# AnnSeidel/genometools

Measured on AMD Instinct MI355X. Metric: Gbp/s ESA build (suf+lcp+bwt), 3 Gbp DNA, 1/2/4/8 MI355X; bit-exact vs CPU, higher is better.
Workload: dtype u64; 1 GPU; human-like DNA (2% N, 24 seqs, repeats) n=3000000000 seed=43 -suf -lcp -bwt (BASELINE.json configs[2]); parallelism=1 device, pair_suffixes=341032298, tied_suffixes=390540711, refine_rounds=9, maxbranchdepth=8256

## Files before the change

genometools_amd/_lib.py:

```python
import ctypes
import os
import subprocess

HERE = os.path.dirname(os.path.abspath(__file__))
ROOT = os.path.dirname(HERE)
LIB_PATH = os.path.join(HERE, "libgtamd_esa.so")
SOURCES = [os.path.join(HERE, "csrc", f) for f in
           ("esa_prims.hip", "esa_engine.hip", "esa_synth.hip", "esa_encode.hip",
            "esa_pck.hip", "esa_comm.hip")]
HEADERS = [os.path.join(HERE, "csrc", f) for f in ("esa_common.h", "esa_prims.h", "esa_devutil.h", "esa_msd.h",
                                                     "esa_pck_replay.h")] + \
          [os.path.join(ROOT, "include", h) for h in ("gtamd_esa.h", "gtamd_encode.h", "gtamd_pck.h")]
HIPCC = os.environ.get("HIPCC", "/opt/rocm/bin/hipcc")


def needs_build():
    if not os.path.exists(LIB_PATH):
        return True
    t = os.path.getmtime(LIB_PATH)
    return any(os.path.getmtime(p) > t for p in SOURCES + HEADERS)


def build_library(force=False, verbose=False):
    if not force and not needs_build():
        return LIB_PATH
    cmd = [HIPCC, "--offload-arch=gfx950", "-O3", "-std=c++17", "-fPIC",
           "-shared", "-Wall", "-Wno-unused-function", "-o", LIB_PATH] + SOURCES
    if verbose:
        print(" ".join(cmd))
    subprocess.run(cmd, check=True)
    return LIB_PATH


class EsaStats(ctypes.Structure):
    _fields_ = [("totallength", ctypes.c_uint64),
                ("numberofallsortedsuffixes", ctypes.c_uint64),
                ("longest", ctypes.c_uint64),
                ("largelcpvalues", ctypes.c_uint64),
                ("maxbranchdepth", ctypes.c_uint64),
                ("lcptabsum", ctypes.c_uint64),
                ("prefixlength", ctypes.c_uint32),
                ("refine_rounds", ctypes.c_uint32),
                ("tied_suffixes", ctypes.c_uint64),
                ("pair_suffixes", ctypes.c_uint64),
                ("device_bytes", ctypes.c_uint64),
                ("msd_big_entries", ctypes.c_uint64),
                ("msd_crowded_entries", ctypes.c_uint64),
                ("rank_entries_built", ctypes.c_uint64)]


class EsaTiming(ctypes.Structure):
    _fields_ = [("total_ms", ctypes.c_float),
                ("keygen_ms", ctypes.c_float),
                ("sort_ms", ctypes.c_float),
                ("finalize_ms", ctypes.c_float),
                ("refine_ms", ctypes.c_float),
                ("tie_fix_ms", ctypes.c_float),
                ("scatter_ms", ctypes.c_float),
                ("scatter_launches", ctypes.c_uint32),
                ("scatter_items", ctypes.c_uint64),
                ("comm_ms", ctypes.c_float),
                ("comm_calls", ctypes.c_uint32),
                ("comm_bytes", ctypes.c_uint64),
                ("alloc_ms", ctypes.c_float),
                ("dominant_kernel", ctypes.c_uint32),
                ("scatter_read_items", ctypes.c_uint64),
                ("scatter_written_items", ctypes.c_uint64)]


class EncodeSummary(ctypes.Structure):
    _fields_ = [(name, ctypes.c_uint64) for name in
                ("totallength", "numofsequences", "specialcharacters",
                 "realspecialranges")] + \
               [("specialrangestab", ctypes.c_uint64 * 3)] + \
               [(name, ctypes.c_uint64) for name in
                ("lengthofspecialprefix", "lengthofspecialsuffix", "wildcards",
                 "realwildcardranges")] + \
               [("wildcardrangestab", ctypes.c_uint64 * 3)] + \
               [(name, ctypes.c_uint64) for name in
                ("lengthofwildcardprefix", "lengthofwildcardsuffix",
                 "lengthoflongestnonspecial", "minseqlen", "maxseqlen",
                 "equallength")] + \
               [("characterdistribution", ctypes.c_uint64 * 32),
                ("originaldistribution", ctypes.c_uint64 * 256)]


class PckParams(ctypes.Structure):
    _fields_ = [("block_size", ctypes.c_uint32), ("bucket_blocks", ctypes.c_uint32),
                ("locate_interval", ctypes.c_uint32), ("feature_toggles", ctypes.c_int32),
                ("with_statistics", ctypes.c_int32)]


class PckInfo(ctypes.Structure):
# ... 115 lines not shown
```

genometools_amd/csrc/esa_engine.hip:

```cpp
#include <stdarg.h>
#include <stdlib.h>
#include <chrono>
#include <functional>
#include <type_traits>
#include <vector>
#include "../../include/gtamd_esa.h"
#include "esa_prims.h"
#include "esa_devutil.h"

static thread_local char g_err[1024] = "";
void gtamd_set_error(const char *fmt, ...) {
  va_list ap;
  va_start(ap, fmt);
  vsnprintf(g_err, sizeof g_err, fmt, ap);
  va_end(ap);
}
extern "C" const char *gtamd_esa_last_error(void) { return g_err; }

extern "C" int gtamd_device_count(void) {
  GTAMD_ABI_BEGIN
  int n = 0;
  if (hipGetDeviceCount(&n) != hipSuccess) return 0;
  return n;
  GTAMD_ABI_END(0)
// ... 2901 lines not shown
  if (m == 0) return 0;
  const u64 nb = div_up(m, 256);
  k_dest_place<F><<<(u32) nb, 256, 0, c->st>>>(f, m, c->numparts, nb, dest, boff);
  HIP_TRY(hipGetLastError());
  return 0;
}
static u64 dest_words(u32 R, u64 m) { return (u64) R * div_up(m ? m : 1, 256) + 16; }

template <int BITS>
static int build_bcktab(gtamd_esa_ctx *c, const u64 *skey, const u32 *spos, u64 NL, u32 k,
                        hipStream_t st) {
  u64 codes = 1, special = 1, dist = 0, pw = 1;
  for (u32 j = 0; j < k; j++) {
    if (codes > (1ull << 31) / c->sigma) {
      gtamd_set_error("bucket table for prefixlength %u over %u letters is too "
                      "large", k, c->sigma);
      return -1;
    }
    codes *= c->sigma;
  }
  for (u32 j = 0; j + 1 < k; j++) special *= c->sigma;
  for (u32 j = 1; j + 1 < k; j++) { pw *= c->sigma; dist += pw; }
  const u64 total = codes + 1 + special + dist;
  free_dev(c->bck);
  c->bck = nullptr;
  HIP_TRY(hipMalloc(&c->bck, total * 4));
  HIP_TRY(hipMemsetAsync(c->bck, 0, total * 4, st));
  if (NL > 0) {
    k_bck_count<BITS><<<(u32) div_up(NL, 256), 256, 0, st>>>(
        skey, NL, k, c->sigma, c->bck, c->bck + codes + 1,
        c->bck + codes + 1 + special, c->text, spos);
    HIP_TRY(hipGetLastError());
  }
  u32 *ws = c->rws.as<u32>();
  u32 *own = nullptr;
  if (scan_workspace_words(codes + 1) * 4 > c->rws.bytes) {
    HIP_TRY(hipMalloc(&own, scan_workspace_words(codes + 1) * 4));
    ws = own;
  }
  const int rc = scan_u32(SCAN_SUM, c->bck, c->bck, codes + 1, false, ws, st);
  if (own != nullptr) { (void) hipStreamSynchronize(st); free_dev(own); }
  TRY(rc);
  c->bck_codes = codes; c->bck_special = special; c->bck_dist = dist;
  return 0;
}

static u64 rws_words_for(u64 cap) {
  return radix_workspace_words(cap) + 10 * (div_up(cap, 64) + 64) +
         scan_workspace_words(div_up(cap, 64)) + 64;
}
static int ensure_workspace(gtamd_esa_ctx *c, u64 cap, u32 want, bool dist) {
  const u64 pad = cap + 8;
  TRY(ensure_buf(c, c->k0, pad * 8, "sort keys"));
  TRY(ensure_buf(c, c->k1, pad * 8, "sort keys"));
  TRY(ensure_buf(c, c->v0, pad * 4, "sort values"));
  TRY(ensure_buf(c, c->v1, pad * 4, "sort values"));
  TRY(ensure_buf(c, c->rws, rws_words_for(cap) * 4, "the radix workspace"));
  TRY(ensure_buf(c, c->tiebits, (div_up(cap, 64) + 2) * 8, "the tie bitmap"));
  if (want & GTAMD_WANT_SUF) TRY(ensure_buf(c, c->suf, pad * 8, "the suffix table"));
  if (want & GTAMD_WANT_LCP) TRY(ensure_buf(c, c->lcp, pad, "the lcp table"));
  if (want & GTAMD_WANT_BWT) TRY(ensure_buf(c, c->bwt, pad, "the bwt table"));
  if (dist) TRY(ensure_buf(c, c->isa_tmp, pad * 8, "the exchange scratch"));
  return 0;
}

static int msd_cbits_max(u64 N) {
  const int c = bits_for(N > 1 ? N - 1 : 1) - 24;
  return c < 0 ? 0 : (c > 8 ? 8 : c);
}
static int msd_choose_cbits(u64 N, int cmax, const float *penalty) {
  int best = cmax;
  float best_cost = 0.0f;
  for (int k = 1; k >= 0; k--) {
    const int c = cmax - 2 + k;
    if (c < 6) continue;
    const float gain = k == 1 ? 0.17f : 0.57f;
    const float cost = (penalty[k] - penalty[2]) / (float) N - gain;
    if (cost < best_cost) { best = c; best_cost = cost; }
  }
  return best;
}
struct MsdWs {
  u32 *hist, *scanws, *tcnt, *tfirst, *dtcnt, *dtfirst, *startA, *startB, *F, *scan2, *counters,
      *biglist, *giantlist, *crowdlist;
  MsTile *desc;
  MdTile *dtiles;
  u64 *firstkey, *lastkey;
  u32 rows, tilesB_ub, tilesC_ub, tilesD_ub;
  u64 nf;
};
static u64 msd_carve(u64 N, int cb, u8 *base, MsdWs *w) {
  const u32 ntA = (u32) div_up(N, MS_TILE);
  w->tilesB_ub = ntA + 256;
  w->tilesC_ub = ntA + MSD_PARENTS;
  w->tilesD_ub = (u32) (2 * div_up(N, MS_TILE)) + MSD_PARENTS + 8;
  w->rows = w->tilesC_ub + 2;
  w->nf = (u64) MSD_PARENTS << cb;
  Bump b;
  b.base = base;
  b.off = 0;
  w->hist = b.take<u32>((u64) w->rows * 256);
  w->scanws = b.take<u32>(radix_rows_workspace_words(w->rows));
  w->desc = b.take<MsTile>(w->tilesC_ub);
  w->tcnt = b.take<u32>(MSD_PARENTS + 8);
  w->tfirst = b.take<u32>(MSD_PARENTS + 8);
  w->dtcnt = b.take<u32>(MSD_PARENTS + 8);
  w->dtfirst = b.take<u32>(MSD_PARENTS + 8);
  w->startA = b.take<u32>(256 + 8);
  w->startB = b.take<u32>(MSD_PARENTS + 8);
  w->F = b.take<u32>(w->nf + 8);
  w->scan2 = b.take<u32>(scan_workspace_words(w->nf + 1) + 64);
  w->counters = b.take<u32>(16);
  w->dtiles = b.take<MdTile>(w->tilesD_ub);
  w->firstkey = b.take<u64>(w->tilesD_ub);
  w->lastkey = b.take<u64>(w->tilesD_ub);
  w->biglist = b.take<u32>(w->tilesD_ub);
  w->crowdlist = b.take<u32>(w->tilesD_ub);
  w->giantlist = b.take<u32>((u64) (N / MS_TILE) + 8);
  return b.off + 256;
}

static int msd_level_prepare(gtamd_esa_ctx *c, const MsdWs &w, const u32 *pstart, u32 np, int cb,
                             u32 tiles_ub, const u32 *kin, u32 *cstart) {
  hipStream_t st = c->st;
  k_msd_tilecount<<<(np + 1 + 255) / 256, 256, 0, st>>>(pstart, 0, np, (u32) MS_TILE, w.tcnt);
  HIP_TRY(hipGetLastError());
  TRY(scan_u32(SCAN_SUM, w.tcnt, w.tfirst, (u64) np + 1, false, w.scan2, st));
  k_msd_tiledesc<<<(tiles_ub + 255) / 256, 256, 0, st>>>(pstart, w.tfirst, np, tiles_ub, w.desc);
  HIP_TRY(hipGetLastError());
  k_msd_hist_lvl<<<tiles_ub + 1, MS_THREADS, 0, st>>>(kin, w.desc, tiles_ub, 32 - cb, w.hist);
  HIP_TRY(hipGetLastError());
  TRY(radix_scan_tile_rows(w.hist, tiles_ub + 1, w.scanws, st));
  const u64 nchild = (u64) np << cb;
  k_msd_tot<<<(u32) div_up(nchild + 1, 256), 256, 0, st>>>(w.hist, w.tfirst, np, cb, cstart);
  HIP_TRY(hipGetLastError());
  TRY(scan_u32(SCAN_SUM, cstart, cstart, nchild + 1, false, w.scan2, st));
  return 0;
}

struct MsdPartSrc {
  const u64 *ck;
  const u32 *cp32;
  u64 index_offset;
  const unsigned long long *prev_key;
  int has_prev;
};
template <int FMT>
static int msd_sort_emit(gtamd_esa_ctx *c, const Switches &sw, u32 want, u32 prefixlength, u64 N,
                         u64 density_n, const MsdPartSrc *src, u32 **sa_out,
                         u64 **fkey, u32 **fval, u64 *local_entries) {
  hipStream_t st = c->st;
  const int cmax = msd_cbits_max(density_n);
  int cb = sw.msd_cbits >= 0 ? sw.msd_cbits : cmax;
  MsdWs w;
  const u64 bytes = msd_carve(N, cb > cmax ? cb : cmax, nullptr, &w);
  TRY(ensure_buf(c, c->msd, bytes, "the tables of the first sort"));
  (void) msd_carve(N, cb > cmax ? cb : cmax, c->msd.as<u8>(), &w);
  const u32 ntA = (u32) div_up(N, MS_TILE);
  const u32 last_valid = (u32) (N - (u64) (ntA - 1) * MS_TILE);
  const u64 pad = N + 8;
  u32 *ka = c->k0.as<u32>(), *pa = c->v0.as<u32>();
  u32 *kb = c->k1.as<u32>(), *pb = c->v1.as<u32>();
  u8 *xa = c->k1.as<u8>() + pad * 4;
  if (src != nullptr)
    k_msd_hist_a_keys<<<ntA, MS_THREADS, 0, st>>>(src->ck, N, w.hist);
  else if (FMT == 1)
    k_msd_hist_a5<<<ntA, MS_THREADS, 0, st>>>(c->text, N, w.hist);
  else
    k_msd_hist_a<<<ntA, MS_THREADS, 0, st>>>(c->text, N, w.hist);
  HIP_TRY(hipGetLastError());
  TRY(radix_scan_tile_rows(w.hist, ntA, w.scanws, st));
  k_msd_starts_a<<<1, 256, 0, st>>>(w.hist, (u32) N, w.startA);
  HIP_TRY(hipGetLastError());
  if (src != nullptr)
    k_msd_scatter_a<1><<<((ntA + 7u) >> 3) * 8u, MS_THREADS, 0, st>>>(
        c->text, N, last_valid, w.hist, ntA, src->ck, src->cp32, ka, xa, pa);
  else if (FMT == 1)
    k_msd_scatter_a<2><<<((ntA + 7u) >> 3) * 8u, MS_THREADS, 0, st>>>(
        c->text, N, last_valid, w.hist, ntA, nullptr, nullptr, ka, xa, pa);
  else
    k_msd_scatter_a<0><<<((ntA + 7u) >> 3) * 8u, MS_THREADS, 0, st>>>(
        c->text, N, last_valid, w.hist, ntA, nullptr, nullptr, ka, xa, pa);
  HIP_TRY(hipGetLastError());
  HIP_TRY(hipEventRecord(c->ev[1], st));
  TRY(msd_level_prepare(c, w, w.startA, 256, 8, w.tilesB_ub, ka, w.startB));
  k_msd_scatter_lvl<1><<<((w.tilesB_ub + 7u) >> 3) * 8u, MS_THREADS, 0, st>>>(
      ka, xa, pa, w.desc, w.tilesB_ub, w.hist, w.tfirst, w.startB, 8, 24, kb, pb);
  HIP_TRY(hipGetLastError());
  if (sw.msd_cbits < 0 && cmax >= 1) {
    float *d_exp = reinterpret_cast<float *>(w.counters);
    float *h_exp = reinterpret_cast<float *>(c->h_counts);
    HIP_TRY(hipMemsetAsync(d_exp, 0, 16, st));
    k_msd_skew<<<MSD_PARENTS / 256, 256, 0, st>>>(w.startB, cmax, d_exp);
    HIP_TRY(hipGetLastError());
    HIP_TRY(hipMemcpyAsync(h_exp, d_exp, 12, hipMemcpyDeviceToHost, st));
    HIP_TRY(hipStreamSynchronize(st));
    cb = msd_choose_cbits(N, cmax, h_exp);
  }
  w.nf = (u64) MSD_PARENTS << cb;
  u32 *kf = kb, *pf = pb, *ko = ka, *po = pa;
  const u32 *F = w.startB;
  if (cb > 0) {
    TRY(msd_level_prepare(c, w, w.startB, MSD_PARENTS, cb, w.tilesC_ub, kb, w.F));
    F = w.F;
    kf = ka; pf = pa; ko = kb; po = pb;
  }
  HIP_TRY(hipMemsetAsync(w.counters, 0, 64, st));
  const u32 pack_cap = sw.msd_pack_cap;
  if (sw.msd_pack) {
    k_msd_pack<false><<<(MSD_PARENTS + 1 + 255) / 256, 256, 0, st>>>(F, cb, nullptr, pack_cap, w.dtcnt, nullptr,
                                                                nullptr, nullptr, nullptr, 0);
    HIP_TRY(hipGetLastError());
    TRY(scan_u32(SCAN_SUM, w.dtcnt, w.dtfirst, (u64) MSD_PARENTS + 1, false, w.scan2, st));
    k_msd_pack<true><<<(MSD_PARENTS + 1 + 255) / 256, 256, 0, st>>>(F, cb, w.dtfirst, pack_cap, nullptr, w.dtiles,
                                                               w.biglist, w.giantlist, w.counters,
                                                               sw.msd_big_max);
    HIP_TRY(hipGetLastError());
  } else {
  k_msd_tilecount<<<(MSD_PARENTS + 1 + 255) / 256, 256, 0, st>>>(F, cb, MSD_PARENTS, MSD_STRIDE,
                                                               w.dtcnt);
  HIP_TRY(hipGetLastError());
  TRY(scan_u32(SCAN_SUM, w.dtcnt, w.dtfirst, (u64) MSD_PARENTS + 1, false, w.scan2, st));
  k_msd_dtiles<<<(w.tilesD_ub + 255) / 256, 256, 0, st>>>(F, cb, w.dtfirst, w.tilesD_ub, w.dtiles,
                                                        w.biglist, w.giantlist, w.crowdlist,
                                                        w.counters, sw.msd_big_max);
  HIP_TRY(hipGetLastError());
  }
  u32 *hc = c->h_counts;
  HIP_TRY(hipMemcpyAsync(hc, w.counters, 16, hipMemcpyDeviceToHost, st));
  HIP_TRY(hipMemcpyAsync(hc + 4, w.dtfirst + MSD_PARENTS, 4, hipMemcpyDeviceToHost, st));
  HIP_TRY(hipStreamSynchronize(st));
  const u32 nbig = hc[0], maxrun = hc[1], nbigentries = hc[2], ngiant = hc[3], ntD = hc[4];
  if (sw.debug)
    fprintf(stderr, "gtamd: msd sort: %d bits at level C, %u runs, %u big (largest %u, %u entries "
            "in all), %u giant\n", cb, ntD, nbig, maxrun, nbigentries, ngiant);
  std::vector<MdTile> giants(ngiant);
  std::vector<u32> giant_t(ngiant);
  if (ngiant > 0) {
    HIP_TRY(hipMemcpy(giant_t.data(), w.giantlist, (size_t) ngiant * 4, hipMemcpyDeviceToHost));
    for (u32 i = 0; i < ngiant; i++)
      HIP_TRY(hipMemcpy(&giants[i], w.dtiles + giant_t[i], sizeof(MdTile), hipMemcpyDeviceToHost));
  }
  if (cb > 0) {
    k_msd_scatter_lvl<2><<<((w.tilesC_ub + 7u) >> 3) * 8u, MS_THREADS, 0, st>>>(
        kb, nullptr, pb, w.desc, w.tilesC_ub, w.hist, w.tfirst, w.F, cb, 32 - cb, ka, pa);
    HIP_TRY(hipGetLastError());
  }
  MsdOut o;
  o.suf = (want & GTAMD_WANT_SUF) ? c->suf.as<u64>() : nullptr;
  o.lcp = (want & GTAMD_WANT_LCP) ? c->lcp.as<u8>() : nullptr;
  o.bwt = (want & GTAMD_WANT_BWT) ? c->bwt.as<u8>() : nullptr;
  o.sa = pf;
  o.tiebits = c->tiebits.as<u64>();
  o.firstkey = w.firstkey;
  o.lastkey = w.lastkey;
  o.stats = c->d_stats;
  o.prefixlength = prefixlength;
  o.index_offset = src != nullptr ? src->index_offset : 0;
  o.val_is_index = src != nullptr && src->cp32 == nullptr;
  if (o.val_is_index) o.suf = nullptr;
  HIP_TRY(hipMemsetAsync(o.tiebits, 0, (div_up(N, 64) + 2) * 8, st));
  if (ntD > 0) {
    HIP_TRY(hipEventRecord(c->ev_scatter[0], st));
    k_msd_local<FMT><<<stride_grid(ntD), MS_THREADS, 0, st>>>(kf, pf, w.dtiles, ntD, cb,
                                                        sw.msd_radix, sw.msd_bin_limit,
                                                        w.crowdlist, w.counters, o);
    HIP_TRY(hipEventRecord(c->ev_scatter[1], st));
    HIP_TRY(hipGetLastError());
    k_msd_local_radix<FMT><<<ntD < 2048u ? ntD : 2048u, MS_THREADS, 0, st>>>(kf, pf, w.dtiles,
                                                                        w.crowdlist, w.counters,
                                                                        cb, o);
    HIP_TRY(hipGetLastError());
  }
  if (nbig > 0) {
    k_msd_big<FMT><<<nbig < 2048u ? nbig : 2048u, MS_THREADS, 0, st>>>(kf, pf, ko, po, w.dtiles,
                                                                w.biglist, w.counters, cb, o);
    HIP_TRY(hipGetLastError());
  }
  for (u32 i = 0; i < ngiant; i++) {
    const MdTile g = giants[i];
    const u64 cnt = g.end - g.begin;
    const int shifts[4] = {FMT == 1 ? 8 : 3, FMT == 1 ? 14 : 11, FMT == 1 ? 20 : 19, FMT == 1 ? 26 : 27};
    const int widths[4] = {FMT == 1 ? 6 : 8, FMT == 1 ? 6 : 8, FMT == 1 ? 6 : 8, FMT == 1 ? 6 : 5};
    int nev = 0;
    TRY(radix_sort_pairs<u32, u32>(kf + g.begin, pf + g.begin, ko + g.begin, po + g.begin, cnt,
                                   shifts, widths, 4, c->rws.as<u32>(), st, nullptr, &nev));
    k_msd_emit_run<FMT><<<(u32) div_up(cnt, MS_TILE), MS_THREADS, 0, st>>>(kf, pf, giant_t[i], g.begin,
                                                                     (u32) cnt, g.s16, o);
    HIP_TRY(hipGetLastError());
  }
  if (ntD > 0) {
    k_msd_seams<FMT><<<(ntD + 255) / 256, 256, 0, st>>>(w.dtiles, ntD, src != nullptr ? src->prev_key : nullptr,
                                                   src != nullptr ? src->has_prev : 0, o);
    HIP_TRY(hipGetLastError());
  }
  *sa_out = pf;
  *fkey = reinterpret_cast<u64 *>(ko);
  *fval = po;
  *local_entries = N - nbigentries;
  c->stats.msd_big_entries = nbigentries;
  return 0;
}

template <int BITS, bool WIDE>
static int run_impl(gtamd_esa_ctx *c, const Switches &sw, u32 want, bool dist) {
  using K = Key<BITS>;
  using P = typename std::conditional<WIDE, u64, u32>::type;
  const u64 N = c->N, n = c->n;
  const u32 R = c->numparts;
  hipStream_t st = c->st;
  const u32 prefixlength = c->user_prefixlength
                               ? c->user_prefixlength
                               : gtamd_recommended_prefixlength(c->sigma, n);
  const bool long_prefix = prefixlength > (u32) K::SYMS;
  if (long_prefix && (want & GTAMD_WANT_LCP)) want |= GTAMD_WANT_SUF;
  const bool want_suf = want & GTAMD_WANT_SUF, want_lcp = want & GTAMD_WANT_LCP,
             want_bwt = want & GTAMD_WANT_BWT;
  if (dist && (want & GTAMD_WANT_BCK)) {
    gtamd_set_error("the bucket table is not available from a part build");
    return -1;
  }
  if (R > 1 && (c->comm_allgather == nullptr || c->comm_alltoallv == nullptr)) {
    gtamd_set_error("a part build needs the collective callbacks "
                    "(gtamd_esa_set_comm)");
    return -1;
  }
  memset(&c->timing, 0, sizeof c->timing);
  memset(&c->stats, 0, sizeof c->stats);
// ... 1442 lines not shown
```

genometools_amd/csrc/esa_msd.h:

```cpp
#pragma once

constexpr int MS_TILE = 4096;
constexpr int MS_THREADS = 512;
constexpr int MS_WAVES = MS_THREADS / 64;
constexpr int MS_ITEMS = MS_TILE / MS_THREADS;
constexpr int MS_WCHUNK = MS_ITEMS * 64;
constexpr int MS_PAD = 520;
constexpr u32 MSD_PARENTS = 65536;
constexpr u32 MSD_STRIDE = 3328;
constexpr int MD_ITEMS = 8;
constexpr u32 MD_CAP = MD_ITEMS * MS_THREADS;
constexpr u32 MSD_BIG_MAX = 1u << 19;

struct MsTile {
  u32 start;
  u32 segvalid;
};
struct MdTile {
  u32 begin, end;
  u32 s16;
  u32 pad;
};
struct MsdOut {
  u64 *suf;
  u8 *lcp;
  u8 *bwt;
  u32 *sa;
  u64 *tiebits;
  u64 *firstkey, *lastkey;
  Stats *stats;
  u32 prefixlength;
  u64 index_offset;
  u32 val_is_index;
};
struct MsdAcc {
  unsigned long long sum, ties;
  u32 mx;
};

__device__ __forceinline__ u32 ms_xcd_tile(u32 b, u32 ntiles) {
  const u32 per = (ntiles + 7u) >> 3;
  return (b & 7u) * per + (b >> 3);
}

template <int FMT> struct MsdFmt;
template <> struct MsdFmt<0> {
  static constexpr int PB = 3;
  static constexpr u32 KSYMS = 20;
};
template <> struct MsdFmt<1> {
  static constexpr int PB = 8;
  static constexpr u32 KSYMS = 8;
};

template <int FMT>
__device__ __forceinline__ u64 msd_full(u32 s16, u32 k2) {
  if (FMT == 1) return ((u64) s16 << 32) | (u64) k2;
  return ((u64) s16 << 48) | ((u64) (k2 >> 8) << 24) | ((u64) ((k2 >> 3) & 31u) << 19) |
         (u64) (k2 & 7u);
}

__device__ __forceinline__ u32 p5_first(u32 pair) { return (pair * 3121u) >> 16; }
__device__ __forceinline__ u32 p5_letters(u64 code) {
#pragma unroll
  for (int k = 0; k < 4; k++) {
    const u32 pr = (u32) (code >> (31 - 9 * k)) & 511u;
    const u32 a = p5_first(pr);
    if (a == 20u) return 2u * k;
    if (pr - 21u * a == 20u) return 2u * k + 1u;
  }
  return ((u32) code & 15u) == 10u ? 8u : 9u;
}
__device__ __forceinline__ u32 p5_common(u64 a, u64 b) {
  const u64 x = a ^ b;
  if ((x >> 4) == 0) return 8u;
  const int lz = __clzll((long long) x) - 24;
  const int f = lz / 9;
  const u32 pa = (u32) (a >> (31 - 9 * f)) & 511u, pb = (u32) (b >> (31 - 9 * f)) & 511u;
  return 2u * (u32) f + (p5_first(pa) == p5_first(pb) ? 1u : 0u);
}
__device__ __forceinline__ u64 p5_code(const Text &t, u64 p, u32 &pay) {
  pay = Pay<5>::before(t, p);
  const u64 win = Sym<5>::window(t, p);
// ... 339 lines not shown
    if (B) atomicAdd(&acc[0], B);
    if (M) atomicMax(&acc[1], (unsigned long long) M);
    if (K) atomicAdd(&acc[2], K);
  }
}

template <typename PV>
__global__ __launch_bounds__(MS_THREADS) void k_part_filter(
    Text t, u64 N, u32 lo, u32 hi, u32 binbelow, const u32 *__restrict__ toff,
    u64 *__restrict__ ck, PV *__restrict__ cp, unsigned long long *__restrict__ prevkey) {
  __shared__ u64 s_k[MS_TILE];
  __shared__ u16 s_off[MS_TILE];
  __shared__ u32 s_scan[MS_WAVES];
  const int tid = threadIdx.x;
  const u64 tile_base = (u64) blockIdx.x * MS_TILE;
  const u64 p0 = tile_base + (u64) tid * KP_PER;
  u64 key[KP_PER];
  u32 mask = 0;
  unsigned long long mx = 0;
  if (p0 < N) {
    const int npos = N - p0 < KP_PER ? (int) (N - p0) : KP_PER;
    dna_keys8(t, p0, key);
#pragma unroll
    for (int g = 0; g < KP_PER; g++) {
      const u32 bin = (u32) (key[g] >> (64 - PART_BITS));
      if (g < npos) {
        if (bin - lo < hi - lo) mask |= 1u << g;
        else if (bin == binbelow) mx = key[g] > mx ? key[g] : mx;
      }
    }
  }
  if (mx) atomicMax(prevkey, mx);
  u32 all;
  u32 at = block_scan_excl<SCAN_SUM, MS_THREADS>((u32) __popc(mask), &all, s_scan);
#pragma unroll
  for (int g = 0; g < KP_PER; g++) {
    if ((mask >> g) & 1u) {
      s_k[at] = key[g];
      s_off[at] = (u16) (tid * KP_PER + g);
      at++;
    }
  }
  __syncthreads();
  const u64 base = toff[blockIdx.x];
  for (u32 i = tid; i < all; i += MS_THREADS) {
    ck[base + i] = s_k[i];
    cp[base + i] = (PV) (tile_base + (u64) s_off[i]);
  }
}

__global__ __launch_bounds__(MS_THREADS) void k_msd_hist_a_keys(const u64 *__restrict__ ck, u64 M,
                                                                u32 *__restrict__ hist) {
  __shared__ u32 h[MS_WAVES][256];
  const int tid = threadIdx.x, w = tid >> 6;
  for (int i = tid; i < MS_WAVES * 256; i += MS_THREADS) (&h[0][0])[i] = 0;
  __syncthreads();
  const u64 base = (u64) blockIdx.x * MS_TILE;
#pragma unroll
  for (int j = 0; j < MS_ITEMS; j++) {
    const u64 e = base + (u64) j * MS_THREADS + tid;
    if (e < M) atomicAdd(&h[w][(u32) (ck[e] >> 56)], 1u);
  }
  __syncthreads();
  if (tid < 256) {
    u32 c = 0;
#pragma unroll
    for (int i = 0; i < MS_WAVES; i++) c += h[i][tid];
    hist[(u64) blockIdx.x * 256 + tid] = c;
  }
}

__global__ __launch_bounds__(256) void k_part_positions(const u32 *__restrict__ idx,
                                                        const u64 *__restrict__ cp, u64 M,
                                                        u64 index_offset, u64 *__restrict__ sa64,
                                                        u64 *__restrict__ suf, Stats *stats) {
  const u64 i = (u64) blockIdx.x * 256 + threadIdx.x;
  if (i >= M) return;
  const u64 p = cp[idx[i]];
  sa64[i] = p;
  if (suf != nullptr) suf[i] = p;
  if (p == 0) stats->longest = index_offset + i;
}

__global__ void k_msd_starts_a(const u32 *__restrict__ scanned, u32 N, u32 *__restrict__ start) {
  const u32 d = threadIdx.x;
  if (d < 256) start[d] = scanned[d];
  if (d == 0) start[256] = N;
}

template <int SRC>
__global__ __launch_bounds__(MS_THREADS) void k_msd_scatter_a(
    Text t, u64 N, u32 last_valid, const u32 *__restrict__ scanned, u32 ntiles,
    const u64 *__restrict__ ck, const u32 *__restrict__ cp32,
    u32 *__restrict__ k1out, u8 *__restrict__ xout, u32 *__restrict__ pout) {
  __shared__ u64 s_t[5120];
  __shared__ u16 s_cnt_mem[MS_WAVES * 256];
  __shared__ u32 s_obase[256];
  __shared__ u32 s_scan[MS_WAVES];
  static_assert(KP_PER * MS_PAD <= 5120 && MS_TILE * 10 <= 5120 * 8, "staging fits");
  const int tid = threadIdx.x, lane = tid & 63, w = tid >> 6;
  const u32 tile = ms_xcd_tile(blockIdx.x, ntiles);
  if (tile >= ntiles) return;
  const u64 tile_base = (u64) tile * MS_TILE;
  const u32 valid = tile + 1u == ntiles ? last_valid : (u32) MS_TILE;
  for (int i = tid; i < MS_WAVES * 256 / 2; i += MS_THREADS)
    reinterpret_cast<u32 *>(s_cnt_mem)[i] = 0;
  u32 gbase = 0;
  if (tid < 256) gbase = scanned[(u64) tile * 256 + tid];
  constexpr bool FROMKEYS = SRC == 1;
  u64 key[MS_ITEMS];
  u32 rk[MS_ITEMS], val[MS_ITEMS];
  if (FROMKEYS) {
#pragma unroll
    for (int j = 0; j < MS_ITEMS; j++) {
      const u32 e = (u32) w * MS_WCHUNK + (u32) j * 64 + lane;
      key[j] = e < valid ? ck[tile_base + e] : ~0ull;
      val[j] = (e < valid && cp32 != nullptr) ? cp32[tile_base + e] : (u32) tile_base + e;
    }
  } else {
  {
    u64 key8[KP_PER];
    const u64 p0 = tile_base + (u64) tid * KP_PER;
    if (p0 < N) {
      if (SRC == 2) p5_keys8(t, p0, key8);
      else dna_keys8(t, p0, key8);
    } else {
#pragma unroll
      for (int g = 0; g < KP_PER; g++) key8[g] = ~0ull;
    }
#pragma unroll
    for (int g = 0; g < KP_PER; g++) s_t[g * MS_PAD + tid] = key8[g];
  }
  __syncthreads();
#pragma unroll
  for (int j = 0; j < MS_ITEMS; j++) {
    const u32 e = (u32) w * MS_WCHUNK + (u32) j * 64 + lane;
    key[j] = s_t[(e & 7u) * MS_PAD + (e >> 3)];
  }
  }
  __syncthreads();
  ms_vu16 *cnt_w = (ms_vu16 *) s_cnt_mem + w * 256;
#pragma unroll
  for (int j = 0; j < MS_ITEMS; j++) {
    const u32 e = (u32) w * MS_WCHUNK + (u32) j * 64 + lane;
    const u32 d = e < valid ? (u32) (key[j] >> 56) : 255u;
    u32 intra, group;
    ms_match<8>(d, intra, group);
    const u32 old = cnt_w[d];
    if (intra == 0) cnt_w[d] = (u16) (old + group);
    rk[j] = ((old + intra) << 8) | d;
  }
  __syncthreads();
  {
    ms_vu16 *s_cnt = (ms_vu16 *) s_cnt_mem;
    u32 c[MS_WAVES];
    u32 tot = 0;
    if (tid < 256) {
#pragma unroll
      for (int i = 0; i < MS_WAVES; i++) {
        c[i] = s_cnt[i * 256 + tid];
        tot += c[i];
      }
    }
    u32 all;
    u32 dbase = block_scan_excl<SCAN_SUM, MS_THREADS>(tot, &all, s_scan);
    if (tid < 256) {
      s_obase[tid] = gbase - dbase;
#pragma unroll
      for (int i = 0; i < MS_WAVES; i++) {
        s_cnt[i * 256 + tid] = (u16) dbase;
        dbase += c[i];
      }
    }
  }
  __syncthreads();
  u32 *s_k1 = reinterpret_cast<u32 *>(s_t);
  u32 *s_p = s_k1 + MS_TILE;
  u8 *s_x = reinterpret_cast<u8 *>(s_p + MS_TILE);
  u8 *s_d = s_x + MS_TILE;
#pragma unroll
  for (int j = 0; j < MS_ITEMS; j++) {
    const u32 e = (u32) w * MS_WCHUNK + (u32) j * 64 + lane;
    const u32 d = rk[j] & 255u;
    const u32 pos = (u32) cnt_w[d] + (rk[j] >> 8);
    s_k1[pos] = (u32) (key[j] >> 24);
    s_p[pos] = FROMKEYS ? val[j] : (u32) tile_base + e;
    s_x[pos] = SRC == 2 ? (u8) ((u32) key[j] & 63u)
                        : (u8) ((((u32) (key[j] >> 19) & 31u) << 3) | ((u32) key[j] & 7u));
    s_d[pos] = (u8) d;
  }
  __syncthreads();
#pragma unroll
  for (int j = 0; j < MS_ITEMS; j++) {
    const u32 e = (u32) j * MS_THREADS + tid;
    if (e < valid) {
      const u32 g = s_obase[s_d[e]] + e;
      k1out[g] = s_k1[e];
      pout[g] = s_p[e];
      xout[g] = s_x[e];
    }
  }
}

__global__ __launch_bounds__(256) void k_msd_tilecount(const u32 *__restrict__ pstart, int sh,
                                                       u32 np, u32 per, u32 *__restrict__ cnt) {
  const u32 s = blockIdx.x * 256u + threadIdx.x;
  if (s > np) return;
  if (s == np) { cnt[s] = 0; return; }
  const u32 size = pstart[(u64) (s + 1) << sh] - pstart[(u64) s << sh];
  cnt[s] = (size + per - 1u) / per;
}

__device__ __forceinline__ u32 ms_parent_of(const u32 *__restrict__ tfirst, u32 np, u32 t) {
  u32 lo = 0, hi = np;
  while (hi - lo > 1) {
    const u32 mid = (lo + hi) >> 1;
    if (tfirst[mid] <= t) lo = mid; else hi = mid;
  }
  return lo;
}

__global__ __launch_bounds__(256) void k_msd_tiledesc(const u32 *__restrict__ pstart,
                                                      const u32 *__restrict__ tfirst, u32 np,
                                                      u32 tiles_ub, MsTile *__restrict__ desc) {
  const u32 t = blockIdx.x * 256u + threadIdx.x;
  if (t >= tiles_ub) return;
  MsTile d;
  d.start = 0;
  d.segvalid = 0;
  if (t < tfirst[np]) {
    const u32 s = ms_parent_of(tfirst, np, t);
    const u32 k = t - tfirst[s];
    const u32 b = pstart[s] + k * (u32) MS_TILE, e = pstart[s + 1];
    const u32 valid = e - b < (u32) MS_TILE ? e - b : (u32) MS_TILE;
    d.start = b;
    d.segvalid = (s << 13) | valid;
  }
  desc[t] = d;
}

__global__ __launch_bounds__(MS_THREADS) void k_msd_hist_lvl(
    const u32 *__restrict__ keys, const MsTile *__restrict__ desc, u32 tiles_ub, int dsh,
    u32 *__restrict__ hist) {
  __shared__ u32 h[MS_WAVES][256];
  const int tid = threadIdx.x, w = tid >> 6;
  for (int i = tid; i < MS_WAVES * 256; i += MS_THREADS) (&h[0][0])[i] = 0;
  __syncthreads();
  const u32 t = blockIdx.x;
  if (t < tiles_ub) {
    const MsTile d = desc[t];
    const u32 valid = d.segvalid & 0x1FFFu;
    u32 head = (4u - (d.start & 3u)) & 3u;
    head = head < valid ? head : valid;
    const u32 nq = (valid - head) >> 2, tail = valid - head - 4u * nq;
    const u32 *kp = keys + d.start;
    uint4 q[2];
#pragma unroll
    for (int j = 0; j < 2; j++) {
      const u32 i = (u32) j * MS_THREADS + tid;
      if (i < nq) q[j] = *reinterpret_cast<const uint4 *>(kp + head + 4u * i);
    }
    if ((u32) tid < head) atomicAdd(&h[w][kp[tid] >> dsh], 1u);
    if ((u32) tid < tail) atomicAdd(&h[w][kp[head + 4u * nq + tid] >> dsh], 1u);
#pragma unroll
    for (int j = 0; j < 2; j++) {
      const u32 i = (u32) j * MS_THREADS + tid;
      if (i < nq) {
        atomicAdd(&h[w][q[j].x >> dsh], 1u);
        atomicAdd(&h[w][q[j].y >> dsh], 1u);
        atomicAdd(&h[w][q[j].z >> dsh], 1u);
        atomicAdd(&h[w][q[j].w >> dsh], 1u);
      }
    }
  }
  __syncthreads();
  if (tid < 256) {
    u32 c = 0;
#pragma unroll
    for (int i = 0; i < MS_WAVES; i++) c += h[i][tid];
    hist[(u64) t * 256 + tid] = c;
  }
}

__global__ __launch_bounds__(256) void k_msd_tot(const u32 *__restrict__ scanned,
                                                 const u32 *__restrict__ tfirst, u32 np, int cb,
                                                 u32 *__restrict__ tot) {
  const u64 i = (u64) blockIdx.x * 256 + threadIdx.x;
  const u64 nchild = (u64) np << cb;
  if (i > nchild) return;
  if (i == nchild) { tot[i] = 0; return; }
  const u32 s = (u32) (i >> cb), d = (u32) i & ((1u << cb) - 1u);
  tot[i] = scanned[(u64) tfirst[s + 1] * 256 + d] - scanned[(u64) tfirst[s] * 256 + d];
}

template <int LEVEL>
__global__ __launch_bounds__(MS_THREADS) void k_msd_scatter_lvl(
    const u32 *__restrict__ kin, const u8 *__restrict__ xin, const u32 *__restrict__ pin,
    const MsTile *__restrict__ desc, u32 tiles_ub, const u32 *__restrict__ scanned,
    const u32 *__restrict__ tfirst, const u32 *__restrict__ cstart, int cb, int dsh,
    u32 *__restrict__ kout, u32 *__restrict__ pout) {
  __shared__ u32 s_key[MS_TILE];
  __shared__ u32 s_val[MS_TILE];
  __shared__ u8 s_x[LEVEL == 1 ? MS_TILE : 4];
  __shared__ u16 s_cnt_mem[MS_WAVES * 256];
  __shared__ u32 s_obase[256];
  __shared__ u32 s_scan[MS_WAVES];
  const int tid = threadIdx.x, lane = tid & 63, w = tid >> 6;
  const u32 tile = ms_xcd_tile(blockIdx.x, tiles_ub);
  if (tile >= tiles_ub) return;
  const MsTile td = desc[tile];
  const u32 valid = td.segvalid & 0x1FFFu, seg = td.segvalid >> 13;
  if (valid == 0) return;
  for (int i = tid; i < MS_WAVES * 256 / 2; i += MS_THREADS)
    reinterpret_cast<u32 *>(s_cnt_mem)[i] = 0;
  u32 gbase = 0;
  if (tid < (1 << cb))
    gbase = cstart[((u64) seg << cb) + tid] + scanned[(u64) tile * 256 + tid] -
            scanned[(u64) tfirst[seg] * 256 + tid];
  u32 key[MS_ITEMS], val[MS_ITEMS], xv[MS_ITEMS], rk[MS_ITEMS];
  const u32 *kp = kin + td.start;
  const u32 *pp = pin + td.start;
  const u8 *xp = xin + td.start;
#pragma unroll
  for (int j = 0; j < MS_ITEMS; j++) {
    const u32 e = (u32) w * MS_WCHUNK + (u32) j * 64 + lane;
    if (e < valid) {
      key[j] = kp[e];
      val[j] = pp[e];
      xv[j] = LEVEL == 1 ? (u32) xp[e] : 0u;
    } else {
      key[j] = ~0u;
      val[j] = 0;
      xv[j] = 0;
    }
  }
  __syncthreads();
  ms_vu16 *cnt_w = (ms_vu16 *) s_cnt_mem + w * 256;
#pragma unroll
  for (int j = 0; j < MS_ITEMS; j++) {
    const u32 e = (u32) w * MS_WCHUNK + (u32) j * 64 + lane;
    const u32 d = e < valid ? key[j] >> dsh : 255u;
    u32 intra, group;
    ms_match<8>(d, intra, group);
    const u32 old = cnt_w[d];
    if (intra == 0) cnt_w[d] = (u16) (old + group);
    rk[j] = ((old + intra) << 8) | d;
  }
  __syncthreads();
  {
    ms_vu16 *s_cnt = (ms_vu16 *) s_cnt_mem;
    u32 c[MS_WAVES];
    u32 tot = 0;
    if (tid < 256) {
#pragma unroll
      for (int i = 0; i < MS_WAVES; i++) {
        c[i] = s_cnt[i * 256 + tid];
        tot += c[i];
      }
    }
    u32 all;
    u32 dbase = block_scan_excl<SCAN_SUM, MS_THREADS>(tot, &all, s_scan);
    if (tid < 256) {
      s_obase[tid] = gbase - dbase;
#pragma unroll
      for (int i = 0; i < MS_WAVES; i++) {
        s_cnt[i * 256 + tid] = (u16) dbase;
        dbase += c[i];
      }
    }
  }
  __syncthreads();
#pragma unroll
  for (int j = 0; j < MS_ITEMS; j++) {
    const u32 d = rk[j] & 255u;
    const u32 pos = (u32) cnt_w[d] + (rk[j] >> 8);
    s_key[pos] = key[j];
    s_val[pos] = val[j];
    if (LEVEL == 1) s_x[pos] = (u8) xv[j];
  }
  __syncthreads();
#pragma unroll
  for (int j = 0; j < MS_ITEMS; j++) {
    const u32 e = (u32) j * MS_THREADS + tid;
    if (e < valid) {
      const u32 k = s_key[e];
      const u32 g = s_obase[k >> dsh] + e;
      kout[g] = LEVEL == 1 ? (k << 8) | (u32) s_x[e] : k;
      pout[g] = s_val[e];
    }
  }
}

__global__ __launch_bounds__(256) void k_msd_skew(const u32 *__restrict__ pstart, int cmax,
                                                  float *__restrict__ out) {
  __shared__ float s_sum[3][4];
  const u32 s = blockIdx.x * 256u + threadIdx.x;
  const float size = s < MSD_PARENTS ? (float) (pstart[s + 1] - pstart[s]) : 0.0f;
  float e[3];
#pragma unroll
  for (int k = 0; k < 3; k++) {
    const int c = cmax - 2 + k;
    float pen = 0.0f;
    if (c >= 0 && size > 0.0f) {
      const float r = size / (float) (1u << c), cap = (float) MD_CAP;
      if (r > 0.95f * cap) pen = 60.0f;
      else if (r >= 1.0f) {
        const float fill = floorf(cap / r) * r / cap;
        pen = 6.0f * (0.85f / fill - 1.0f);
        if (pen < 0.0f) pen = 0.0f;
      }
    }
    e[k] = size * pen;
  }
#pragma unroll
  for (int k = 0; k < 3; k++) {
    float v = e[k];
    for (int d = 32; d >= 1; d >>= 1) v += __shfl_xor(v, d, 64);
    if ((threadIdx.x & 63) == 0) s_sum[k][threadIdx.x >> 6] = v;
  }
  __syncthreads();
  if (threadIdx.x < 3) {
    const float t = s_sum[threadIdx.x][0] + s_sum[threadIdx.x][1] + s_sum[threadIdx.x][2] +
                    s_sum[threadIdx.x][3];
    if (t > 0.0f) atomicAdd(&out[threadIdx.x], t);
  }
}

__global__ __launch_bounds__(256) void k_msd_dtiles(const u32 *__restrict__ F, int cb,
                                                    const u32 *__restrict__ tfirst, u32 tiles_ub,
                                                    MdTile *__restrict__ tiles,
                                                    u32 *__restrict__ biglist,
                                                    u32 *__restrict__ giantlist,
                                                    u32 *__restrict__ crowdlist,
                                                    u32 *__restrict__ counters, u32 big_max) {
  const u32 t = blockIdx.x * 256u + threadIdx.x;
  if (t >= tiles_ub) return;
  MdTile d;
  d.begin = d.end = d.s16 = d.pad = 0;
  if (t < tfirst[MSD_PARENTS]) {
    const u32 s = ms_parent_of(tfirst, MSD_PARENTS, t);
    const u32 k = t - tfirst[s], count = tfirst[s + 1] - tfirst[s];
    const u64 lo = (u64) s << cb, hi = (u64) (s + 1) << cb;
    const u32 pbase = F[lo];
    u32 cut[2];
    u64 cutj[2];
#pragma unroll
    for (int q = 0; q < 2; q++) {
      const u32 kk = k + (u32) q;
      if (kk == 0) { cut[q] = pbase; cutj[q] = lo; }
      else if (kk >= count) { cut[q] = F[hi]; cutj[q] = hi; }
      else {
        const u64 target = (u64) pbase + (u64) kk * MSD_STRIDE;
        u64 a = lo, b = hi;
        while (b - a > 1) {
          const u64 mid = (a + b) >> 1;
          if ((u64) F[mid] >= target) b = mid; else a = mid;
        }
        cut[q] = F[b];
// ... 708 lines not shown
```

Baseline: 25.07 Gbp/s.

## Pack first-level MSD scatter output into u64 entries with block-relative positions

For text-sourced first sorts, the level-A scatter now writes a single packed u64 per suffix (32-bit key, 8-bit extra symbol, 24-bit low position) instead of three separate key/extra/position arrays. The full position is rebuilt in level B from per-bucket block boundaries: a binary search over boundaries computed by an extended starts kernel, with the level histogram templated to read the u64 keys. The aim is fewer scattered writes and reads in the first two passes. In exchange it adds boundary bookkeeping, a per-element search, and depends on a 24-bit position field holding for the chosen block size.

```diff
diff --git a/genometools_amd/_lib.py b/genometools_amd/_lib.py
--- a/genometools_amd/_lib.py
+++ b/genometools_amd/_lib.py
@@ -8,7 +8,7 @@
 SOURCES = [os.path.join(HERE, "csrc", f) for f in
            ("esa_prims.hip", "esa_engine.hip", "esa_synth.hip", "esa_encode.hip",
             "esa_pck.hip", "esa_comm.hip")]
-HEADERS = [os.path.join(HERE, "csrc", f) for f in ("esa_common.h", "esa_prims.h", "esa_devutil.h", "esa_msd.h",
+HEADERS = [os.path.join(HERE, "csrc", f) for f in ("esa_common.h", "esa_prims.h", "esa_devutil.h", "esa_msd.h", "esa_msd_blocks.h",
                                                      "esa_pck_replay.h")] + \
           [os.path.join(ROOT, "include", h) for h in ("gtamd_esa.h", "gtamd_encode.h", "gtamd_pck.h")]
 HIPCC = os.environ.get("HIPCC", "/opt/rocm/bin/hipcc")
diff --git a/genometools_amd/csrc/esa_engine.hip b/genometools_amd/csrc/esa_engine.hip
--- a/genometools_amd/csrc/esa_engine.hip
+++ b/genometools_amd/csrc/esa_engine.hip
@@ -3007,7 +3007,7 @@
 }
 struct MsdWs {
   u32 *hist, *scanws, *tcnt, *tfirst, *dtcnt, *dtfirst, *startA, *startB, *F, *scan2, *counters,
-      *biglist, *giantlist, *crowdlist;
+      *biglist, *giantlist, *crowdlist, *bndA;
   MsTile *desc;
   MdTile *dtiles;
   u64 *firstkey, *lastkey;
@@ -3032,6 +3032,7 @@
   w->dtcnt = b.take<u32>(MSD_PARENTS + 8);
   w->dtfirst = b.take<u32>(MSD_PARENTS + 8);
   w->startA = b.take<u32>(256 + 8);
+  w->bndA = b.take<u32>(256 * MSD_BLOCKS);
   w->startB = b.take<u32>(MSD_PARENTS + 8);
   w->F = b.take<u32>(w->nf + 8);
   w->scan2 = b.take<u32>(scan_workspace_words(w->nf + 1) + 64);
@@ -3046,14 +3047,17 @@
 }
 
 static int msd_level_prepare(gtamd_esa_ctx *c, const MsdWs &w, const u32 *pstart, u32 np, int cb,
-                             u32 tiles_ub, const u32 *kin, u32 *cstart) {
+                             u32 tiles_ub, const u32 *kin, const u64 *ein, u32 *cstart) {
   hipStream_t st = c->st;
   k_msd_tilecount<<<(np + 1 + 255) / 256, 256, 0, st>>>(pstart, 0, np, (u32) MS_TILE, w.tcnt);
   HIP_TRY(hipGetLastError());
   TRY(scan_u32(SCAN_SUM, w.tcnt, w.tfirst, (u64) np + 1, false, w.scan2, st));
   k_msd_tiledesc<<<(tiles_ub + 255) / 256, 256, 0, st>>>(pstart, w.tfirst, np, tiles_ub, w.desc);
   HIP_TRY(hipGetLastError());
-  k_msd_hist_lvl<<<tiles_ub + 1, MS_THREADS, 0, st>>>(kin, w.desc, tiles_ub, 32 - cb, w.hist);
+  if (ein != nullptr)
+    k_msd_hist_lvl<u64><<<tiles_ub + 1, MS_THREADS, 0, st>>>(ein, w.desc, tiles_ub, 32 - cb, w.hist);
+  else
+    k_msd_hist_lvl<u32><<<tiles_ub + 1, MS_THREADS, 0, st>>>(kin, w.desc, tiles_ub, 32 - cb, w.hist);
   HIP_TRY(hipGetLastError());
   TRY(radix_scan_tile_rows(w.hist, tiles_ub + 1, w.scanws, st));
   const u64 nchild = (u64) np << cb;
@@ -3087,6 +3091,9 @@
   u32 *ka = c->k0.as<u32>(), *pa = c->v0.as<u32>();
   u32 *kb = c->k1.as<u32>(), *pb = c->v1.as<u32>();
   u8 *xa = c->k1.as<u8>() + pad * 4;
+  u64 *ea = c->k0.as<u64>();
+  const bool wide = src == nullptr;
+  const int lbits = msd_block_bits(N);
   if (src != nullptr)
     k_msd_hist_a_keys<<<ntA, MS_THREADS, 0, st>>>(src->ck, N, w.hist);
   else if (FMT == 1)
@@ -3095,22 +3102,29 @@
     k_msd_hist_a<<<ntA, MS_THREADS, 0, st>>>(c->text, N, w.hist);
   HIP_TRY(hipGetLastError());
   TRY(radix_scan_tile_rows(w.hist, ntA, w.scanws, st));
-  k_msd_starts_a<<<1, 256, 0, st>>>(w.hist, (u32) N, w.startA);
+  k_msd_starts_a<<<wide ? MSD_BLOCKS : 1, 256, 0, st>>>(w.hist, (u32) N, ntA, lbits, w.startA,
+                                                         wide ? w.bndA : nullptr);
   HIP_TRY(hipGetLastError());
   if (src != nullptr)
     k_msd_scatter_a<1><<<((ntA + 7u) >> 3) * 8u, MS_THREADS, 0, st>>>(
-        c->text, N, last_valid, w.hist, ntA, src->ck, src->cp32, ka, xa, pa);
+        c->text, N, last_valid, w.hist, ntA, src->ck, src->cp32, ka, xa, pa, nullptr);
   else if (FMT == 1)
     k_msd_scatter_a<2><<<((ntA + 7u) >> 3) * 8u, MS_THREADS, 0, st>>>(
-        c->text, N, last_valid, w.hist, ntA, nullptr, nullptr, ka, xa, pa);
+        c->text, N, last_valid, w.hist, ntA, nullptr, nullptr, nullptr, nullptr, nullptr, ea);
   else
     k_msd_scatter_a<0><<<((ntA + 7u) >> 3) * 8u, MS_THREADS, 0, st>>>(
-        c->text, N, last_valid, w.hist, ntA, nullptr, nullptr, ka, xa, pa);
+        c->text, N, last_valid, w.hist, ntA, nullptr, nullptr, nullptr, nullptr, nullptr, ea);
   HIP_TRY(hipGetLastError());
   HIP_TRY(hipEventRecord(c->ev[1], st));
-  TRY(msd_level_prepare(c, w, w.startA, 256, 8, w.tilesB_ub, ka, w.startB));
-  k_msd_scatter_lvl<1><<<((w.tilesB_ub + 7u) >> 3) * 8u, MS_THREADS, 0, st>>>(
-      ka, xa, pa, w.desc, w.tilesB_ub, w.hist, w.tfirst, w.startB, 8, 24, kb, pb);
+  TRY(msd_level_prepare(c, w, w.startA, 256, 8, w.tilesB_ub, ka, wide ? ea : nullptr, w.startB));
+  if (wide)
+    k_msd_scatter_lvl<1, true><<<((w.tilesB_ub + 7u) >> 3) * 8u, MS_THREADS, 0, st>>>(
+        nullptr, nullptr, nullptr, ea, w.bndA, lbits, w.desc, w.tilesB_ub, w.hist, w.tfirst,
+        w.startB, 8, 24, kb, pb);
+  else
+    k_msd_scatter_lvl<1, false><<<((w.tilesB_ub + 7u) >> 3) * 8u, MS_THREADS, 0, st>>>(
+        ka, xa, pa, nullptr, nullptr, 0, w.desc, w.tilesB_ub, w.hist, w.tfirst, w.startB, 8, 24,
+        kb, pb);
   HIP_TRY(hipGetLastError());
   if (sw.msd_cbits < 0 && cmax >= 1) {
     float *d_exp = reinterpret_cast<float *>(w.counters);
@@ -3126,7 +3140,7 @@
   u32 *kf = kb, *pf = pb, *ko = ka, *po = pa;
   const u32 *F = w.startB;
   if (cb > 0) {
-    TRY(msd_level_prepare(c, w, w.startB, MSD_PARENTS, cb, w.tilesC_ub, kb, w.F));
+    TRY(msd_level_prepare(c, w, w.startB, MSD_PARENTS, cb, w.tilesC_ub, kb, nullptr, w.F));
     F = w.F;
     kf = ka; pf = pa; ko = kb; po = pb;
   }
@@ -3167,8 +3181,9 @@
       HIP_TRY(hipMemcpy(&giants[i], w.dtiles + giant_t[i], sizeof(MdTile), hipMemcpyDeviceToHost));
   }
   if (cb > 0) {
-    k_msd_scatter_lvl<2><<<((w.tilesC_ub + 7u) >> 3) * 8u, MS_THREADS, 0, st>>>(
-        kb, nullptr, pb, w.desc, w.tilesC_ub, w.hist, w.tfirst, w.F, cb, 32 - cb, ka, pa);
+    k_msd_scatter_lvl<2, false><<<((w.tilesC_ub + 7u) >> 3) * 8u, MS_THREADS, 0, st>>>(
+        kb, nullptr, pb, nullptr, nullptr, 0, w.desc, w.tilesC_ub, w.hist, w.tfirst, w.F, cb,
+        32 - cb, ka, pa);
     HIP_TRY(hipGetLastError());
   }
   MsdOut o;
diff --git a/genometools_amd/csrc/esa_msd.h b/genometools_amd/csrc/esa_msd.h
--- a/genometools_amd/csrc/esa_msd.h
+++ b/genometools_amd/csrc/esa_msd.h
@@ -1,4 +1,5 @@
 #pragma once
+#include "esa_msd_blocks.h"
 
 constexpr int MS_TILE = 4096;
 constexpr int MS_THREADS = 512;
@@ -504,22 +505,33 @@
   if (p == 0) stats->longest = index_offset + i;
 }
 
-__global__ void k_msd_starts_a(const u32 *__restrict__ scanned, u32 N, u32 *__restrict__ start) {
-  const u32 d = threadIdx.x;
-  if (d < 256) start[d] = scanned[d];
-  if (d == 0) start[256] = N;
+__global__ __launch_bounds__(256) void k_msd_starts_a(const u32 *__restrict__ scanned, u32 N,
+                                                      u32 ntiles, int L, u32 *__restrict__ start,
+                                                      u32 *__restrict__ bnd) {
+  const u32 d = threadIdx.x, k = blockIdx.x;
+  if (k == 0) {
+    start[d] = scanned[d];
+    if (d == 0) start[256] = N;
+  }
+  if (bnd != nullptr) {
+    const u32 t = k << (L - 12);
+    const u32 end = d < 255u ? scanned[d + 1] : N;
+    bnd[d * MSD_BLOCKS + k] = t < ntiles ? scanned[(u64) t * 256 + d] : end;
+  }
 }
 
 template <int SRC>
 __global__ __launch_bounds__(MS_THREADS) void k_msd_scatter_a(
     Text t, u64 N, u32 last_valid, const u32 *__restrict__ scanned, u32 ntiles,
     const u64 *__restrict__ ck, const u32 *__restrict__ cp32,
-    u32 *__restrict__ k1out, u8 *__restrict__ xout, u32 *__restrict__ pout) {
+    u32 *__restrict__ k1out, u8 *__restrict__ xout, u32 *__restrict__ pout,
+    u64 *__restrict__ eout) {
   __shared__ u64 s_t[5120];
   __shared__ u16 s_cnt_mem[MS_WAVES * 256];
   __shared__ u32 s_obase[256];
   __shared__ u32 s_scan[MS_WAVES];
-  static_assert(KP_PER * MS_PAD <= 5120 && MS_TILE * 10 <= 5120 * 8, "staging fits");
+  static_assert(KP_PER * MS_PAD <= 5120 && MS_TILE * 10 <= 5120 * 8 && MS_TILE * 9 <= 5120 * 8,
+                "staging fits");
   const int tid = threadIdx.x, lane = tid & 63, w = tid >> 6;
   const u32 tile = ms_xcd_tile(blockIdx.x, ntiles);
   if (tile >= ntiles) return;
@@ -596,6 +608,26 @@
     }
   }
   __syncthreads();
+  if (!FROMKEYS) {
+    u8 *s_d = reinterpret_cast<u8 *>(s_t + MS_TILE);
+#pragma unroll
+    for (int j = 0; j < MS_ITEMS; j++) {
+      const u32 e = (u32) w * MS_WCHUNK + (u32) j * 64 + lane;
+      const u32 d = rk[j] & 255u;
+      const u32 pos = (u32) cnt_w[d] + (rk[j] >> 8);
+      const u32 x = SRC == 2 ? (u32) key[j] & 63u
+                             : (((u32) (key[j] >> 19) & 31u) << 3) | ((u32) key[j] & 7u);
+      s_t[pos] = ((key[j] >> 24) << 32) | ((u64) x << 24) | (u64) (((u32) tile_base + e) & 0xFFFFFFu);
+      s_d[pos] = (u8) d;
+    }
+    __syncthreads();
+#pragma unroll
+    for (int j = 0; j < MS_ITEMS; j++) {
+      const u32 e = (u32) j * MS_THREADS + tid;
+      if (e < valid) eout[s_obase[s_d[e]] + e] = s_t[e];
+    }
+    return;
+  }
   u32 *s_k1 = reinterpret_cast<u32 *>(s_t);
   u32 *s_p = s_k1 + MS_TILE;
   u8 *s_x = reinterpret_cast<u8 *>(s_p + MS_TILE);
@@ -661,9 +693,16 @@
   desc[t] = d;
 }
 
+template <typename KT>
+__device__ __forceinline__ u32 ms_hist_key(KT k) {
+  return sizeof(KT) == 8 ? (u32) ((u64) k >> 32) : (u32) k;
+}
+template <typename KT>
 __global__ __launch_bounds__(MS_THREADS) void k_msd_hist_lvl(
-    const u32 *__restrict__ keys, const MsTile *__restrict__ desc, u32 tiles_ub, int dsh,
+    const KT *__restrict__ keys, const MsTile *__restrict__ desc, u32 tiles_ub, int dsh,
     u32 *__restrict__ hist) {
+  constexpr u32 PER = 16 / sizeof(KT);
+  constexpr int NLD = MS_TILE / (int) PER / MS_THREADS;
   __shared__ u32 h[MS_WAVES][256];
   const int tid = threadIdx.x, w = tid >> 6;
   for (int i = tid; i < MS_WAVES * 256; i += MS_THREADS) (&h[0][0])[i] = 0;
@@ -672,25 +711,27 @@
   if (t < tiles_ub) {
     const MsTile d = desc[t];
     const u32 valid = d.segvalid & 0x1FFFu;
-    u32 head = (4u - (d.start & 3u)) & 3u;
+    u32 head = (PER - (d.start & (PER - 1u))) & (PER - 1u);
     head = head < valid ? head : valid;
-    const u32 nq = (valid - head) >> 2, tail = valid - head - 4u * nq;
-    const u32 *kp = keys + d.start;
-    uint4 q[2];
-#pragma unroll
-    for (int j = 0; j < 2; j++) {
+    const u32 nq = (valid - head) / PER, tail = valid - head - PER * nq;
+    const KT *kp = keys + d.start;
+    uint4 q[NLD];
+#pragma unroll
+    for (int j = 0; j < NLD; j++) {
       const u32 i = (u32) j * MS_THREADS + tid;
-      if (i < nq) q[j] = *reinterpret_cast<const uint4 *>(kp + head + 4u * i);
-    }
-    if ((u32) tid < head) atomicAdd(&h[w][kp[tid] >> dsh], 1u);
-    if ((u32) tid < tail) atomicAdd(&h[w][kp[head + 4u * nq + tid] >> dsh], 1u);
-#pragma unroll
-    for (int j = 0; j < 2; j++) {
+      if (i < nq) q[j] = *reinterpret_cast<const uint4 *>(kp + head + PER * i);
+    }
+    if ((u32) tid < head) atomicAdd(&h[w][ms_hist_key(kp[tid]) >> dsh], 1u);
+    if ((u32) tid < tail) atomicAdd(&h[w][ms_hist_key(kp[head + PER * nq + tid]) >> dsh], 1u);
+#pragma unroll
+    for (int j = 0; j < NLD; j++) {
       const u32 i = (u32) j * MS_THREADS + tid;
       if (i < nq) {
-        atomicAdd(&h[w][q[j].x >> dsh], 1u);
+        if (PER == 4) {
+          atomicAdd(&h[w][q[j].x >> dsh], 1u);
+          atomicAdd(&h[w][q[j].z >> dsh], 1u);
+        }
         atomicAdd(&h[w][q[j].y >> dsh], 1u);
-        atomicAdd(&h[w][q[j].z >> dsh], 1u);
         atomicAdd(&h[w][q[j].w >> dsh], 1u);
       }
     }
@@ -715,18 +756,22 @@
   tot[i] = scanned[(u64) tfirst[s + 1] * 256 + d] - scanned[(u64) tfirst[s] * 256 + d];
 }
 
-template <int LEVEL>
+template <int LEVEL, bool WIDE>
 __global__ __launch_bounds__(MS_THREADS) void k_msd_scatter_lvl(
     const u32 *__restrict__ kin, const u8 *__restrict__ xin, const u32 *__restrict__ pin,
+    const u64 *__restrict__ ein, const u32 *__restrict__ bnd, int lbits,
     const MsTile *__restrict__ desc, u32 tiles_ub, const u32 *__restrict__ scanned,
     const u32 *__restrict__ tfirst, const u32 *__restrict__ cstart, int cb, int dsh,
     u32 *__restrict__ kout, u32 *__restrict__ pout) {
+  static_assert(!WIDE || LEVEL == 1, "only level A writes the u64 entries");
   __shared__ u32 s_key[MS_TILE];
   __shared__ u32 s_val[MS_TILE];
   __shared__ u8 s_x[LEVEL == 1 ? MS_TILE : 4];
   __shared__ u16 s_cnt_mem[MS_WAVES * 256];
   __shared__ u32 s_obase[256];
   __shared__ u32 s_scan[MS_WAVES];
+  __shared__ u32 s_in[WIDE ? MSD_BLOCKS : 1];
+  __shared__ u32 s_bcnt[WIDE ? 8 : 1];
   const int tid = threadIdx.x, lane = tid & 63, w = tid >> 6;
   const u32 tile = ms_xcd_tile(blockIdx.x, tiles_ub);
   if (tile >= tiles_ub) return;
@@ -735,25 +780,51 @@
   if (valid == 0) return;
   for (int i = tid; i < MS_WAVES * 256 / 2; i += MS_THREADS)
     reinterpret_cast<u32 *>(s_cnt_mem)[i] = 0;
+  u32 bk = 0;
+  if (WIDE && tid >= 1 && tid < MSD_BLOCKS) bk = bnd[seg * MSD_BLOCKS + tid];
   u32 gbase = 0;
   if (tid < (1 << cb))
     gbase = cstart[((u64) seg << cb) + tid] + scanned[(u64) tile * 256 + tid] -
             scanned[(u64) tfirst[seg] * 256 + tid];
   u32 key[MS_ITEMS], val[MS_ITEMS], xv[MS_ITEMS], rk[MS_ITEMS];
-  const u32 *kp = kin + td.start;
-  const u32 *pp = pin + td.start;
-  const u8 *xp = xin + td.start;
-#pragma unroll
-  for (int j = 0; j < MS_ITEMS; j++) {
-    const u32 e = (u32) w * MS_WCHUNK + (u32) j * 64 + lane;
-    if (e < valid) {
-      key[j] = kp[e];
-      val[j] = pp[e];
-      xv[j] = LEVEL == 1 ? (u32) xp[e] : 0u;
-    } else {
-      key[j] = ~0u;
-      val[j] = 0;
-      xv[j] = 0;
+  if (WIDE) {
+    u64 en[MS_ITEMS];
+#pragma unroll
+    for (int j = 0; j < MS_ITEMS; j++) {
+      const u32 e = (u32) w * MS_WCHUNK + (u32) j * 64 + lane;
+      en[j] = e < valid ? ein[td.start + e] : ~0ull << 32;
+    }
+#pragma unroll
+    for (int j = 0; j < MS_ITEMS; j++) {
+      key[j] = (u32) (en[j] >> 32);
+      xv[j] = (u32) (en[j] >> 24) & 255u;
+      val[j] = (u32) en[j] & 0xFFFFFFu;
+    }
+  } else {
+    const u32 *kp = kin + td.start;
+    const u32 *pp = pin + td.start;
+    const u8 *xp = xin + td.start;
+#pragma unroll
+    for (int j = 0; j < MS_ITEMS; j++) {
+      const u32 e = (u32) w * MS_WCHUNK + (u32) j * 64 + lane;
+      if (e < valid) {
+        key[j] = kp[e];
+        val[j] = pp[e];
+        xv[j] = LEVEL == 1 ? (u32) xp[e] : 0u;
+      } else {
+        key[j] = ~0u;
+        val[j] = 0;
+        xv[j] = 0;
+      }
+    }
+  }
+  u32 bcls = 0;
+  if (WIDE) {
+    if (tid >= 1 && tid < MSD_BLOCKS) bcls = msd_bound_class(bk, td.start, valid);
+    const u64 b1 = __ballot(bcls == 1u), b2 = __ballot(bcls == 2u);
+    if (lane == 0 && w < MSD_BLOCKS / 64) {
+      s_bcnt[2 * w] = (u32) __popcll(b1);
+      s_bcnt[2 * w + 1] = (u32) __popcll(b2);
     }
   }
   __syncthreads();
@@ -768,6 +839,16 @@
     if (intra == 0) cnt_w[d] = (u16) (old + group);
     rk[j] = ((old + intra) << 8) | d;
   }
+  u32 kb0 = 0, nin = 0;
+  if (WIDE) {
+#pragma unroll
+    for (int i = 0; i < MSD_BLOCKS / 64; i++) {
+      kb0 += s_bcnt[2 * i];
+      nin += s_bcnt[2 * i + 1];
+    }
+    const u32 at = (u32) tid - 1u - kb0;
+    if (bcls == 2u && at < (u32) MSD_BLOCKS) s_in[at] = bk - td.start;
+  }
   __syncthreads();
   {
     ms_vu16 *s_cnt = (ms_vu16 *) s_cnt_mem;
@@ -796,6 +877,11 @@
   for (int j = 0; j < MS_ITEMS; j++) {
     const u32 d = rk[j] & 255u;
     const u32 pos = (u32) cnt_w[d] + (rk[j] >> 8);
+    if (WIDE) {
+      const u32 e = (u32) w * MS_WCHUNK + (u32) j * 64 + lane;
+      const u32 blk = nin == 0 ? kb0 : msd_block_in_tile(kb0, s_in, nin, e);
+      val[j] = msd_position(blk, val[j], lbits);
+    }
     s_key[pos] = key[j];
     s_val[pos] = val[j];
     if (LEVEL == 1) s_x[pos] = (u8) xv[j];
diff --git a/genometools_amd/csrc/esa_msd_blocks.h b/genometools_amd/csrc/esa_msd_blocks.h
--- /dev/null
+++ b/genometools_amd/csrc/esa_msd_blocks.h
@@ -0,0 +1,47 @@
+#pragma once
+#include <stdint.h>
+
+#if defined(__HIPCC__)
+#define MSD_HD __host__ __device__ __forceinline__
+#else
+#define MSD_HD inline
+#endif
+
+constexpr int MSD_BLOCKS = 256;
+
+MSD_HD int msd_block_bits(uint64_t N) {
+  int c = 0;
+  while (c < 40 && (1ull << c) < N) c++;
+  c -= 8;
+  return c < 12 ? 12 : (c > 24 ? 24 : c);
+}
+
+MSD_HD uint32_t msd_bound_class(uint32_t b, uint32_t start, uint32_t valid) {
+  return b <= start ? 1u : (b - start < valid ? 2u : 0u);
+}
+
+template <typename P>
+MSD_HD uint32_t msd_block_in_tile(uint32_t kb0, P in, uint32_t m, uint32_t e) {
+  uint32_t lo = 0, hi = m;
+  while (lo < hi) {
+    const uint32_t mid = (lo + hi) >> 1;
+    if (in[mid] <= e) lo = mid + 1; else hi = mid;
+  }
+  return kb0 + lo;
+}
+
+MSD_HD uint32_t msd_position(uint32_t block, uint32_t low24, int L) {
+  return (block << L) | (low24 & ((1u << L) - 1u));
+}
+
+inline uint32_t msd_tile_bounds(const uint32_t *row, uint32_t start, uint32_t valid,
+                                uint32_t *in, uint32_t *m) {
+  uint32_t kb0 = 0;
+  *m = 0;
+  for (int k = 1; k < MSD_BLOCKS; k++) {
+    const uint32_t c = msd_bound_class(row[k], start, valid);
+    if (c == 1u) kb0++;
+    if (c == 2u) in[(*m)++] = row[k] - start;
+  }
+  return kb0;
+}
```

Measured after the change: 26.03 Gbp/s, median of 6. +3.8%, better.
